# lms-07/LGTEUN

Hardware: AMD Instinct MI355X
Metric: train image-pairs/sec, GF-2 4-band 128x128, K=4, bs=32/GPU (higher is better)
Workload: dtype f32 (GEMMs and the local mixer: split 16-bit MFMA -- f16 pairs in the forward FFN, the W2 products of its backward and P V, bf16 triples elsewhere -- fp32 accumulate; fp32-equivalent); 1 GPU; BASELINE configs[1]: C=4, MS 32x32, PAN 128x128, K=4, 32 pairs/GPU, train step = fwd + L1 + bwd + Adam + StepLR tick; mode=faithful, global_batch=32, parallelism=dp1, dropout=True

## Files before the change

### include/lgteun_hip.h

```cpp
#ifndef LGTEUN_HIP_H
#define LGTEUN_HIP_H

#include <stddef.h>
#include <stdint.h>

#ifdef __cplusplus
extern "C" {
#endif

#define LG_TENSORS_SHARED 12
#define LG_TENSORS_PER_STAGE 119

#define LG_FLAG_FAITHFUL 1
#define LG_FLAG_SAVE 2
#define LG_FLAG_DROPOUT 4

#define LG_FLAG_BWD_LGT 8
#define LG_FLAG_BWD_DATA 16

#define LG_FLAG_CHAINED 32

#define LG_FLAG_DEFER_DEAD 64

#define LG_FLAG_STAGEWISE 128
// ... 83 lines not shown

int lg_optim_step_ex(float* params, const float* grads, float* state0, float* state1, float* state2, const int64_t* ranges,
                     int32_t n_ranges, int64_t max_range, int32_t step, int32_t algo, int32_t flags, double lr, double h0, double h1,
                     double eps, double weight_decay, double grad_scale, const float* clip_coef, float* ema, double ema_decay,
                     int32_t plain_adam, void* stream);

int lg_prof_enable(int32_t kernel_id, int32_t max_launches);
int lg_prof_reset(void);
void lg_prof_pause(int32_t paused);
int lg_prof_read(double* total_ms, int64_t* launches);
void lg_prof_disable(void);
const char* lg_kernel_name(int32_t kernel_id);

int lg_dropout_mask(uint64_t seed, int32_t stage, int32_t blk, int64_t first, int64_t n, float* out, void* stream);

int lg_op_resample(const float* x, float* y, int32_t planes, int32_t hi, int32_t wi, int32_t mode, void* stream);
int lg_op_data_step(const lg_plan* plan, const float* params, int32_t stage, const float* z_in, const float* ms,
                    const float* pan, float* z_out, float* tmp, int32_t B, void* stream);
int lg_op_lgt(const lg_plan* plan, const float* params, int32_t stage, const float* z, float* out, void* workspace,
              size_t workspace_bytes, int32_t B, int32_t flags, uint64_t seed, void* stream);
int lg_op_lgt_stages(const lg_plan* plan, const float* params, int32_t stage0, int32_t n, const float* z, float* out, void* workspace,
                     size_t workspace_bytes, int32_t B, int32_t flags, uint64_t seed, int32_t grid_cap, void* stream);
int lg_workspace_deadout(const lg_plan* plan, int32_t B, int32_t train, size_t* offset, size_t* stage_stride);
int lg_op_block(const lg_plan* plan, const float* params, int32_t stage, int32_t blk, int32_t which, const float* x,
                float* y, void* workspace, size_t workspace_bytes, int32_t B, void* stream);

int lg_op_block_bwd(const lg_plan* plan, const float* params, float* grads, int32_t stage, int32_t blk, int32_t which,
                    const float* x, const float* dy, float* dx, void* workspace, size_t workspace_bytes, int32_t B,
                    void* stream);

int lg_op_data_step_bwd(const lg_plan* plan, const float* params, float* grads, int32_t stage, const float* z_in, const float* ms,
                        const float* pan, const float* dz_out, float* dz_in, void* workspace, size_t workspace_bytes, int32_t B,
                        void* stream);
int lg_op_lgt_bwd(const lg_plan* plan, const float* params, float* grads, int32_t stage, const float* z, const float* dout, float* dz,
                  void* workspace, size_t workspace_bytes, int32_t B, int32_t flags, uint64_t seed, void* stream);

#define LG_IQA_PEAK 2047.5
#define LG_IQA_SSIM_TAPS 11
#define LG_IQA_SSIM_SIGMA 1.5
#define LG_IQA_Q_BLOCK 8
#define LG_IQA_RATIO 4
#define LG_IQA_QNR_BLOCK 32
#define LG_IQA_MTF_TAPS 41
#define LG_IQA_MTF_GAIN 0.15
#define LG_IQA_MAX_BANDS 16
size_t lg_iqa_workspace_bytes(int32_t B, int32_t C, int32_t H, int32_t W, int32_t no_ref);
// ... 31 lines not shown
```

### lgteun_amd/_lib.py

```python
import ctypes
import os
from ctypes import POINTER, c_char_p, c_double, c_float, c_int32, c_int64, c_size_t, c_uint64, c_void_p

_HERE = os.path.dirname(os.path.abspath(__file__))
LIB_PATH = os.environ.get('LGTEUN_HIP_LIB') or os.path.join(_HERE, '_lgteun_hip.so')

LG_FLAG_FAITHFUL = 1
LG_FLAG_SAVE = 2
LG_FLAG_DROPOUT = 4
LG_FLAG_BWD_LGT = 8
LG_FLAG_BWD_DATA = 16
LG_FLAG_CHAINED = 32
LG_FLAG_DEFER_DEAD = 64
LG_FLAG_STAGEWISE = 128
KERNEL_IDS = {n: i for i, n in enumerate(['none', 'ffn1', 'ffn', 'fft', 'attn', 'upfuse', 'down', 'embed', 'tail', 'datastep', 'ffn1_bwd',
                                           'ffn2_bwd', 'fft_bwd', 'attn_bwd', 'wgrad', 'batch', 'scene_gather', 'scene_blend'])}


class LgConfig(ctypes.Structure):
    _fields_ = [('C', c_int32), ('K', c_int32), ('H', c_int32), ('W', c_int32), ('precision', c_int32), ('variant', ctypes.c_uint32)]


LG_VAR_FFN_STRIP, LG_VAR_FFN_TILE, LG_VAR_FFN_XP = 1, 2, 3
LG_VAR_FFN_SAVE3, LG_VAR_FFN_SAVE5 = 1 << 2, 2 << 2
# ... 67 lines not shown
    'lgteun_forward': (c_int32, [c_void_p, c_void_p, c_void_p, c_void_p, c_void_p, c_void_p, c_size_t, c_int32, c_int32,
                                 c_uint64, c_void_p]),
    'lgteun_backward': (c_int32, [c_void_p, c_void_p, c_void_p, c_void_p, c_void_p, c_void_p, c_void_p, c_size_t, c_int32,
                                  c_int32, c_uint64, c_void_p]),
    'lgteun_dead_forward': (c_int32, [c_void_p, c_void_p, c_void_p, c_size_t, c_int32, c_int32, c_uint64, c_void_p]),
    'lg_l1_loss': (c_int32, [c_void_p, c_void_p, c_void_p, c_void_p, c_int64, c_int64, c_float, c_void_p]),
    'lg_adam_step': (c_int32, [c_void_p, c_void_p, c_void_p, c_void_p, c_void_p, c_int32, c_int64, c_int32, c_float, c_float,
                               c_float, c_float, c_float, c_void_p]),
    'lg_l2_loss': (c_int32, [c_void_p, c_void_p, c_void_p, c_void_p, c_int64, c_int64, c_float, c_void_p]),
    'lg_optim_step': (c_int32, [c_void_p, c_void_p, c_void_p, c_void_p, c_void_p, c_void_p, c_int32, c_int64, c_int32, c_int32, c_int32,
                                c_double, c_double, c_double, c_double, c_double, c_double, c_void_p]),
    'lg_grad_norm_workspace_bytes': (c_size_t, [c_int32, c_int64]),
    'lg_grad_norm': (c_int32, [c_void_p, c_void_p, c_int32, c_int64, c_double, c_void_p, c_void_p, c_size_t, c_void_p]),
    'lg_optim_step_ex': (c_int32, [c_void_p, c_void_p, c_void_p, c_void_p, c_void_p, c_void_p, c_int32, c_int64, c_int32, c_int32, c_int32,
                                   c_double, c_double, c_double, c_double, c_double, c_double, c_void_p, c_void_p, c_double, c_int32,
                                   c_void_p]),
    'lg_op_resample': (c_int32, [c_void_p, c_void_p, c_int32, c_int32, c_int32, c_int32, c_void_p]),
    'lg_op_data_step': (c_int32, [c_void_p, c_void_p, c_int32, c_void_p, c_void_p, c_void_p, c_void_p, c_void_p, c_int32,
                                  c_void_p]),
    'lg_op_lgt': (c_int32, [c_void_p, c_void_p, c_int32, c_void_p, c_void_p, c_void_p, c_size_t, c_int32, c_int32, c_uint64,
                            c_void_p]),
    'lg_op_lgt_stages': (c_int32, [c_void_p, c_void_p, c_int32, c_int32, c_void_p, c_void_p, c_void_p, c_size_t, c_int32, c_int32, c_uint64,
                                   c_int32, c_void_p]),
    'lg_workspace_deadout': (c_int32, [c_void_p, c_int32, c_int32, POINTER(c_size_t), POINTER(c_size_t)]),
    'lg_op_block': (c_int32, [c_void_p, c_void_p, c_int32, c_int32, c_int32, c_void_p, c_void_p, c_void_p, c_size_t, c_int32,
                              c_void_p]),
    'lg_dropout_mask': (c_int32, [c_uint64, c_int32, c_int32, c_int64, c_int64, c_void_p, c_void_p]),
    'lg_prof_enable': (c_int32, [c_int32, c_int32]),
    'lg_prof_reset': (c_int32, []),
    'lg_prof_pause': (None, [c_int32]),
    'lg_prof_read': (c_int32, [POINTER(ctypes.c_double), POINTER(c_int64)]),
    'lg_prof_disable': (None, []),
    'lg_kernel_name': (c_char_p, [c_int32]),
    'lg_op_data_step_bwd': (c_int32, [c_void_p, c_void_p, c_void_p, c_int32, c_void_p, c_void_p, c_void_p, c_void_p, c_void_p, c_void_p,
                                      c_size_t, c_int32, c_void_p]),
    'lg_op_lgt_bwd': (c_int32, [c_void_p, c_void_p, c_void_p, c_int32, c_void_p, c_void_p, c_void_p, c_void_p, c_size_t, c_int32, c_int32,
                                c_uint64, c_void_p]),
    'lg_op_block_bwd': (c_int32, [c_void_p, c_void_p, c_void_p, c_int32, c_int32, c_int32, c_void_p, c_void_p, c_void_p, c_void_p,
                                  c_size_t, c_int32, c_void_p]),
    'lg_iqa_workspace_bytes': (c_size_t, [c_int32, c_int32, c_int32, c_int32, c_int32]),
    'lg_iqa_ref': (c_int32, [c_void_p, c_void_p, c_void_p, c_int32, c_int32, c_int32, c_int32, c_float, c_void_p, c_size_t, c_void_p]),
    'lg_iqa_no_ref': (c_int32, [c_void_p, c_void_p, c_void_p, c_void_p, c_int32, c_int32, c_int32, c_int32, c_float, c_void_p, c_size_t,
                                c_void_p]),
    'lg_pyr_down2': (c_int32, [c_void_p, c_void_p, c_int64, c_int32, c_int32, c_int32, c_void_p]),
    'lg_batch_assemble': (c_int32, [c_void_p, c_void_p, c_void_p, c_void_p, c_int64, c_void_p, c_int64, c_void_p, c_void_p, c_void_p, c_void_p,
                                    c_void_p, c_int32, c_int32, c_int32, c_int32, c_int32, c_int32, c_int32, c_float, c_int32, c_float, c_void_p]),
# ... 34 lines not shown
```

### lgteun_amd/csrc/api.hip

```cpp
#include <stdarg.h>
#include <stdio.h>
#include <stdlib.h>
#include <string.h>
#include <math.h>
#include <atomic>
#include <mutex>

#pragma GCC visibility push(default)
#include "../../include/lgteun_hip.h"
#pragma GCC visibility pop

#include "kernels.h"
#include "workspace.h"
#include "backward.h"

static thread_local char g_err[512] = "";

void lg_set_error(const char* fmt, ...) {
    va_list ap;
    va_start(ap, fmt);
    vsnprintf(g_err, sizeof(g_err), fmt, ap);
    va_end(ap);
}

// ... 442 lines not shown
}

extern "C" int lg_op_lgt(const lg_plan* plan, const float* params, int32_t stage, const float* z, float* out, void* workspace,
                         size_t workspace_bytes, int32_t B, int32_t flags, uint64_t seed, void* stream) {
    if (!plan || !params || !z || !out || !workspace || stage < 0 || stage >= plan->cfg.K) { lg_set_error("op_lgt: invalid argument"); return -1; }
    const int train = (flags & LG_FLAG_SAVE) ? 1 : 0;
    if (workspace_bytes < lg_workspace_bytes(plan, B, train)) { lg_set_error("op_lgt: workspace too small"); return -3; }
    NetBufs nb;
    carve(plan, B, train, workspace, nb);
    return lgt_fwd(plan, params, stage, z, out, nb, B, flags, seed, (hipStream_t)stream);
}

extern "C" int lg_op_lgt_stages(const lg_plan* plan, const float* params, int32_t stage0, int32_t n, const float* z, float* out, void* workspace,
                                size_t workspace_bytes, int32_t B, int32_t flags, uint64_t seed, int32_t grid_cap, void* stream) {
    if (!plan || !params || !z || !out || !workspace || B <= 0 || stage0 < 0 || n < 1 || stage0 + n > plan->cfg.K || grid_cap < 0) { lg_set_error("op_lgt_stages: invalid argument"); return -1; }
    if (flags & ~LG_FLAG_DROPOUT) { lg_set_error("op_lgt_stages: only LG_FLAG_DROPOUT applies (nothing is saved)"); return -2; }
    if (n > 1 && (!plan->stage_batch || n > plan->cfg.K - 1)) { lg_set_error("op_lgt_stages: this plan runs one stage per pass (lg_plan_stage_batch), or n > K-1"); return -2; }
    if (workspace_bytes < lg_workspace_bytes(plan, B, 0)) { lg_set_error("op_lgt_stages: workspace too small"); return -3; }
    NetBufs nb;
    carve(plan, B, 0, workspace, nb);
    hipStream_t s = (hipStream_t)stream;
    if (int rc = prep_stages(plan, params, stage0, stage0 + n, nb, s)) return rc;
    return lgt_fwd(plan, params, stage0, z, out, nb, B, flags, seed, s, true, n, (long)B * plan->cfg.C * plan->cfg.H * plan->cfg.W, grid_cap);
}

extern "C" int lg_op_block(const lg_plan* plan, const float* params, int32_t stage, int32_t blk, int32_t which, const float* x,
                           float* y, void* workspace, size_t workspace_bytes, int32_t B, void* stream) {
    if (!plan || !params || !x || !y || !workspace || stage < 0 || stage >= plan->cfg.K || blk < 0 || blk > 4 || which < 0 || which > 2) {
        lg_set_error("op_block: invalid argument");
        return -1;
    }
    if (workspace_bytes < lg_workspace_bytes(plan, B, 0)) { lg_set_error("op_block: workspace too small"); return -3; }
    hipStream_t s = (hipStream_t)stream;
    NetBufs nb;
    carve(plan, B, 0, workspace, nb);
    BlockBufs bb = nb.blk[blk];
    int rc;
    const size_t npix = (size_t)B * bb.h * bb.w;
    if (which == 0 || which == 1) {
        if ((rc = launch_ln_split(bb.e, x, params + plan->blk(stage, blk, B_LN1G), params + plan->blk(stage, blk, B_LN1B), bb.g, B,
                                  bb.h * bb.w, s)))
            return rc;
    }
    if (which == 0) {
        FftArgs f;
        f.g = bb.g; f.o = y; f.amp = nullptr; f.pha = nullptr; f.sgn = nullptr; f.scratch = nb.fft_scratch;
// ... 467 lines not shown
```

### lgteun_amd/csrc/k_attn_m.hip

```cpp
#include "kernels.h"
#include "split_bf16.h"


namespace am {

__host__ __device__ constexpr int pw(int prod) { return prod == 0 ? 1 : prod == 1 ? 1 : prod == 2 ? 2 : prod == 3 ? 1 : prod == 4 ? 3 : 2; }
__host__ __device__ constexpr int px(int prod) { return prod == 0 ? 1 : prod == 1 ? 2 : prod == 2 ? 1 : prod == 3 ? 3 : prod == 4 ? 1 : 2; }
__host__ __device__ constexpr int pw2(int prod) { return prod == 0 ? 2 : 1; }
__host__ __device__ constexpr int px2(int prod) { return prod == 1 ? 2 : 1; }
__host__ __device__ constexpr int nprod(int np) { return np == 3 ? 6 : (np == 2 ? 3 : 1); }
template <int NP> __host__ __device__ constexpr int pwN(int prod) { return NP == 2 ? pw2(prod) : pw(prod); }
template <int NP> __host__ __device__ constexpr int pxN(int prod) { return NP == 2 ? px2(prod) : px(prod); }
__host__ __device__ constexpr int cdiv(int a, int b) { return (a + b - 1) / b; }

__device__ __forceinline__ float vmax2(float a, float b) { return fmaxf(a, b); }
__device__ __forceinline__ float vmax3(float a, float b, float c) { return fmaxf(fmaxf(a, b), c); }
__device__ __forceinline__ float xg_sum(float v) {
    u32x2_t r = __builtin_amdgcn_permlane32_swap(__float_as_uint(v), __float_as_uint(v), false, false);
    v = __uint_as_float(r.x) + __uint_as_float(r.y);
    r = __builtin_amdgcn_permlane16_swap(__float_as_uint(v), __float_as_uint(v), false, false);
    return __uint_as_float(r.x) + __uint_as_float(r.y);
}
__device__ __forceinline__ float xg_max(float v) {
    u32x2_t r = __builtin_amdgcn_permlane32_swap(__float_as_uint(v), __float_as_uint(v), false, false);
// ... 120 lines not shown

template <int HC>
struct Geo {
    static constexpr int E = 2 * HC, D = HC / 2, DG = D / 4;
    static constexpr int NCH = E / 16;
    static constexpr int NY = HC >= 16 ? HC / 16 : 1;
    static constexpr int MTQK = D / 4;
    static constexpr int NTV = HC >= 16 ? HC / 16 : 1;
    __host__ __device__ static constexpr int qk_oc(int mt, int r) {
        const int gq = r >> 2, idx = mt * 4 + (r & 3);
        const int isq = idx / (2 * DG), h = (idx / DG) % 2, dd = idx % DG;
        return (isq ? 0 : HC) + h * D + gq * DG + dd;
    }
    __host__ __device__ static constexpr int v_oc(int nt, int c) { return (HC == 8 && c >= 8) ? -1 : 2 * HC + 16 * nt + c; }
};

}

#ifdef LG_ATTN_STAMPS
__device__ unsigned long long am_stamps[1024][4][8];
#define AM_STAMP(i) do { __builtin_amdgcn_sched_barrier(0); const unsigned long long t__ = __builtin_amdgcn_s_memtime(); st[i] += t__ - tprev; tprev = t__; __builtin_amdgcn_sched_barrier(0); } while (0)
#else
#define AM_STAMP(i) do { } while (0)
#endif
template <int HC, int NP, bool MULTI = false>
__global__ __launch_bounds__(256, (HC <= 16 ? 2 : 1)) void k_attn_m(AttnArgs a_, int nwin, int nquads, int uneven) {
    using namespace am;
    using G = Geo<HC>;
    constexpr int E = G::E, D = G::D, DG = G::DG, NCH = G::NCH, NY = G::NY, MTQK = G::MTQK, NTV = G::NTV;
    constexpr int NPQ = NP == 2 ? 2 : NP, NPP = NP == 2 ? 3 : NP;
    constexpr int CHY = 4 * NY, NKQ = cdiv(nprod(NPQ) * CHY, 8);
    constexpr int NKS = cdiv(nprod(NPQ) * DG, 8);
    constexpr int CHC = 4 * NCH, NKP = cdiv(nprod(NPP) * CHC, 8);
    constexpr int MTP = NCH;
    constexpr int NPV = NP >= 2 ? 2 : 1;
    constexpr bool RELOADX = HC >= 32;
    constexpr float LOG2E = 1.44269504088896340736f;
    extern __shared__ __attribute__((aligned(16))) u32x4_t smem4[];
    float4* sPos = reinterpret_cast<float4*>(smem4);
    u32x4_t* sWqk = smem4 + 2 * 4 * 4 * 64;
    u32x4_t* sWv = sWqk + MTQK * NKQ * 64;
    u32x4_t* sWp = sWv + NTV * NKQ * 64;
    const int lane = threadIdx.x & 63, wave = threadIdx.x >> 6, g = lane >> 4, c = lane & 15;

#ifdef LG_ATTN_STAMPS
    unsigned long long st[8] = {0, 0, 0, 0, 0, 0, 0, 0}, tprev = __builtin_amdgcn_s_memtime();
#endif
    const StageSel sg = a_.sg;
    constexpr bool multi = MULTI;
    const int half = (int)gridDim.x >> 1, first = (int)blockIdx.x < half ? 1 : 0;
    const int nmine = uneven ? (first ? uneven : 8 - uneven) : 0x7fffffff;
    const int q0 = uneven ? (first ? (int)blockIdx.x : half * uneven + ((int)blockIdx.x - half)) : (int)blockIdx.x;
    const int qstep = multi ? 1 : (uneven ? half : (int)gridDim.x);
    const int per_stage = multi ? __builtin_amdgcn_readfirstlane(nquads / sg.n) : nquads;
    const int run0 = multi ? __builtin_amdgcn_readfirstlane((int)(blockIdx.x * (unsigned)nquads / gridDim.x)) : q0;
    const int run1 = multi ? __builtin_amdgcn_readfirstlane((int)((blockIdx.x + 1) * (unsigned)nquads / gridDim.x)) : nquads;
    int seg0 = run0;
    do {
    const int stg = multi ? __builtin_amdgcn_readfirstlane(seg0 / per_stage) : 0;
    const int seg1 = multi ? min(run1, (stg + 1) * per_stage) : run1;
    AttnArgs a = a_;
    {
        const long po = stg * sg.pstride;
        a.pos += po; a.ln1g += po; a.ln1b += po; a.qkvw += po; a.qkvb += po; a.projw += po; a.projb += po;
        if (NP == 2) a.scales += stg * sg.as_stride;
    }
    const uint64_t dseed = multi ? mix_seed(sg.seed, sg.stage0 + stg, sg.blk) : a.seed;
    const long dpix0 = (long)stg * sg.Bs * a.h * a.w;
    if (seg0 != run0) __syncthreads();
    float sy = 1.f, sw = 1.f, sq = 1.f, sk = 1.f;
    if (NP == 2) { sy = uniform_f(a.scales[0]); sw = uniform_f(a.scales[1]); sq = uniform_f(a.scales[2]); sk = uniform_f(a.scales[3]); }
    const float syw = sy * sw, inv_yw = 1.0f / syw, sqk = sq * sk, inv_qk = 1.0f / sqk;
    float4 pv[8];
#pragma unroll
    for (int j = 0; j < 8; ++j) {
        const int u = j * 256 + threadIdx.x, ln = u & 63, kt = (u >> 6) & 3, qt = (u >> 8) & 3, h = u >> 10;
        pv[j] = *reinterpret_cast<const float4*>(a.pos + ((h * 64 + 16 * qt + (ln & 15)) * 64 + 16 * kt + 4 * (ln >> 4)));
    }
    auto oc_qk = [](int t, int r) { return G::qk_oc(t, r); };
    auto oc_v = [](int t, int r) { return G::v_oc(t, r); };
    auto oc_p = [](int t, int r) { return 16 * t + r; };
    WStage<NPQ, CHY, NKQ, MTQK> wsq;
    WStage<NPQ, CHY, NKQ, NTV> wsv;
// ... 237 lines not shown
            for (int mt = 0; mt < MTP; ++mt) {
                f32x4_t acc = {bp[mt][0], bp[mt][1], bp[mt][2], bp[mt][3]};
#pragma unroll
                for (int k = 0; k < NKP; ++k) acc = mfma_bf(sWp[(mt * NKP + k) * 64 + lane], cf[k], acc);
                float o[4];
                const uint64_t di = (uint64_t)((pix - dpix0) * E + 16 * mt + 4 * g);
#pragma unroll
                for (int v = 0; v < 4; ++v) o[v] = acc[v];
                if (a.dropout) {
                    float s0, s1, s2, s3;
                    dropout_scale2(dseed, di, s0, s1);
                    dropout_scale2(dseed, di + 2, s2, s3);
                    o[0] *= s0; o[1] *= s1; o[2] *= s2; o[3] *= s3;
                }
                const float4 xr = RELOADX ? *reinterpret_cast<const float4*>(xw + (qt * tstep * E + 16 * mt + lx)) : xv[qt][mt];
                *reinterpret_cast<float4*>(yw + (qt * tstep * E + 16 * mt + lx)) = make_float4(xr.x + o[0], xr.y + o[1], xr.z + o[2], xr.w + o[3]);
            }
        }
        AM_STAMP(5);
    }
    seg0 = seg1;
    } while (MULTI && seg0 < run1);
#ifdef LG_ATTN_STAMPS
    if (lane == 0 && blockIdx.x < 1024) {
        for (int i = 0; i < 6; ++i) am_stamps[blockIdx.x][wave][i] = st[i];
        am_stamps[blockIdx.x][wave][7] = 1ull;
    }
#endif
}

template <int HC, int NP, bool MULTI = false>
static int launch_attn_m_t(const AttnArgs& a, hipStream_t s) {
    using G = am::Geo<HC>;
    constexpr int NPQ = NP == 2 ? 2 : NP, NPP = NP == 2 ? 3 : NP;
    constexpr int NKQ = am::cdiv(am::nprod(NPQ) * 4 * G::NY, 8), NKP = am::cdiv(am::nprod(NPP) * 4 * G::NCH, 8);
    const int nwin = a.B * (a.h / 8) * (a.w / 8);
    const int nquads = (nwin + 3) / 4;
    const size_t lds = (size_t)(2 * 4 * 4 * 64 + (G::MTQK + G::NTV) * NKQ * 64 + G::NCH * NKP * 64) * 16;
    static DeviceOnce attr_once;
    if (attr_once.need()) {
        hipError_t e = hipFuncSetAttribute((const void*)k_attn_m<HC, NP, MULTI>, hipFuncAttributeMaxDynamicSharedMemorySize, 160 * 1024);
        if (e != hipSuccess) { lg_set_error("attn_m: hipFuncSetAttribute: %s", hipGetErrorString(e)); return (int)e; }
        attr_once.done();
    }
    static std::atomic<int> per_cu_cache[64];
    int per_cu = per_cu_cache[DeviceOnce::dev()].load(std::memory_order_acquire);
    if (per_cu <= 0) {
        int nb = 0;
        hipError_t e = hipOccupancyMaxActiveBlocksPerMultiprocessor(&nb, (const void*)k_attn_m<HC, NP, MULTI>, 256, lds);
        if (e != hipSuccess || nb < 1) { lg_set_error("attn_m: occupancy query: %s (%d)", hipGetErrorString(e), nb); return e != hipSuccess ? (int)e : -3; }
        per_cu = nb;
        per_cu_cache[DeviceOnce::dev()].store(per_cu, std::memory_order_release);
    }
    int ncu = 256;
    const int cap = ncu * per_cu;
    const int rounds = (nquads + cap - 1) / cap;
    int grid = nquads < cap ? nquads : (nquads + rounds - 1) / rounds;
    constexpr bool multi = MULTI;
    if (multi) {
        if (a.save_o || a.save_l || a.sg.Bs <= 0 || a.B != a.sg.n * a.sg.Bs || (a.sg.Bs * (a.h / 8) * (a.w / 8)) % 4) { lg_set_error("attn_m: a window quad would straddle the stages of the launch"); return -2; }
        if (nquads > cap) grid = cap;
        if (a.sg.grid_cap > 0 && grid > a.sg.grid_cap) grid = a.sg.grid_cap;
    }
#ifndef LG_ATTN_UNEVEN
#define LG_ATTN_UNEVEN 5
#endif
    const int uneven = (!multi && per_cu == 2 && grid == 512 && nquads == 4 * grid && nwin == 4 * nquads) ? LG_ATTN_UNEVEN : 0;
    k_attn_m<HC, NP, MULTI><<<grid, 256, lds, s>>>(a, nwin, nquads, uneven == 4 ? 0 : uneven);
    LG_CHECK_LAUNCH();
    return 0;
}

int launch_attn_m(int e, const AttnArgs& a, hipStream_t s) {
    ProfScope prof__(LG_K_ATTN, s, a.sg.n);
    if ((a.h & 7) || (a.w & 7)) { lg_set_error("attn: h,w must be multiples of 8"); return -2; }
    if (a.sg.n > 1) {
        if (e == 16) return a.bf16 ? launch_attn_m_t<8, 1, true>(a, s) : (a.scales ? launch_attn_m_t<8, 2, true>(a, s) : launch_attn_m_t<8, 3, true>(a, s));
        if (e == 32) return a.bf16 ? launch_attn_m_t<16, 1, true>(a, s) : (a.scales ? launch_attn_m_t<16, 2, true>(a, s) : launch_attn_m_t<16, 3, true>(a, s));
        lg_set_error("attn: e=%d takes one stage per launch", e);
        return -2;
    }
    if (a.bf16) {
        if (e == 16) return launch_attn_m_t<8, 1>(a, s);
        if (e == 32) return launch_attn_m_t<16, 1>(a, s);
        if (e == 64) return launch_attn_m_t<32, 1>(a, s);
    } else if (a.scales) {
        if (e == 16) return launch_attn_m_t<8, 2>(a, s);
        if (e == 32) return launch_attn_m_t<16, 2>(a, s);
        if (e == 64) return launch_attn_m_t<32, 2>(a, s);
    } else {
        if (e == 16) return launch_attn_m_t<8, 3>(a, s);
// ... 7 lines not shown
```

### lgteun_amd/csrc/k_ffn_xr.hip

```cpp
#include "kernels.h"

#include "hstore.h"
#include "split_bf16.h"

#ifndef LG_XR_GRID
#define LG_XR_GRID 512
#endif
#ifdef LG_STAMPS
__device__ unsigned long long g_xr_stamps[512 * 4 * 10 * 8];
#define XSTAMP_AT(si_, i) do { unsigned long long t__; asm volatile("s_memtime %0\n\ts_waitcnt lgkmcnt(0)" : "=s"(t__)); \
                       g_xr_stamps[(((blockIdx.x & 511) * 4 + wave) * 10 + (si_)) * 8 + (i)] = t__; } while (0)
#define XSTAMP(i) do { unsigned long long t__; asm volatile("s_memtime %0\n\ts_waitcnt lgkmcnt(0)" : "=s"(t__)); \
                       g_xr_stamps[(((blockIdx.x & 511) * 4 + wave) * 10 + (stamp_si < 9 ? stamp_si : 9)) * 8 + (i)] = t__; } while (0)
extern "C" __attribute__((visibility("default"))) int lg_debug_xr_stamps(unsigned long long* host) {
    return (int)hipMemcpyFromSymbol(host, HIP_SYMBOL(g_xr_stamps), sizeof(g_xr_stamps));
}
#else
#define XSTAMP_AT(si_, i) do { } while (0)
#define XSTAMP(i) do { } while (0)
#endif

#ifndef LG_XR_TURN
#define LG_XR_TURN 0
#endif
#ifndef LG_XR_UNEVEN
#define LG_XR_UNEVEN 16
#endif
#define XR_TAKE_TURNS() do { if (LG_XR_TURN) { \
        const unsigned long long tt__ = __builtin_amdgcn_s_memtime(); \
        if ((((unsigned)(tt__ >> LG_XR_TURN)) ^ slot_par) & 1u) __builtin_amdgcn_s_setprio(3); else __builtin_amdgcn_s_setprio(0); } } while (0)
__device__ unsigned g_xr_turn[8192];

namespace xr {

constexpr int E = 16, N1 = 64, TX = 16, HX = 18, TY = 8, RING = 10, LDR = 68;
constexpr int NF1 = 8, NF2 = 16, NF3 = 4, NFRAG = NF1 + NF2 + NF3;
constexpr size_t OFF_W = 0;
constexpr size_t OFF_TAPS = OFF_W + (size_t)NFRAG * 64 * 16;
constexpr size_t OFF_PAR = OFF_TAPS + (size_t)N1 * 9 * 4;
constexpr int P_B1 = 0, P_B2 = 64, P_DWB = 128, P_B3 = 192, P_N1G = 208, P_N1B = 224, P_FLOATS = 240;
constexpr size_t OFF_RING = OFF_PAR + (size_t)P_FLOATS * 4;
constexpr size_t LDS_BYTES = OFF_RING + (size_t)RING * HX * LDR * 4;
static_assert(LDS_BYTES <= 80 * 1024, "two workgroups per CU");
static_assert(OFF_RING % 16 == 0 && OFF_TAPS % 16 == 0 && OFF_PAR % 16 == 0, "16-byte aligned LDS regions");

#ifndef LG_XR_NT
#define LG_XR_NT 0
#endif
#ifndef LG_XR_FENCES
// ... 63 lines not shown
template <int SAVE, int NP, bool MULTI = false>
__global__ __launch_bounds__(256) __attribute__((amdgpu_waves_per_eu(2))) void k_ffn_xr(Ffn1Args a1_, Ffn2Args a2_, int tiles_x, int strips_y, int nstrips,
                                                                                       int SH, int dS) {
    using namespace xr;
    extern __shared__ __attribute__((aligned(16))) unsigned char smem_raw[];
    float* ring = reinterpret_cast<float*>(smem_raw + OFF_RING);
    u32x4_t* sW = reinterpret_cast<u32x4_t*>(smem_raw + OFF_W);
    float* sTaps = reinterpret_cast<float*>(smem_raw + OFF_TAPS);
    float* sPar = reinterpret_cast<float*>(smem_raw + OFF_PAR);
    const int wave = threadIdx.x >> 6, lane = threadIdx.x & 63, g = lane >> 4, c_ = lane & 15, c = c_;
    const int uwave = __builtin_amdgcn_readfirstlane(wave);
    unsigned slot_par = 0;
    if (LG_XR_TURN) {
        const unsigned hw = __builtin_amdgcn_s_getreg((12 - 1) << 11 | 4 << 6 | 4);
        const unsigned xcc = __builtin_amdgcn_s_getreg((3 - 1) << 11 | 0 << 6 | 20);
        const unsigned key = (xcc << 10) | (((hw >> 9) & 7u) << 7) | (((hw >> 8) & 1u) << 6) | (((hw >> 4) & 15u) << 2) | (hw & 3u);
        unsigned old_ = 0;
        if (lane == 0) old_ = atomicXor(&g_xr_turn[key & 8191u], 1u);
        slot_par = (unsigned)__builtin_amdgcn_readfirstlane((int)old_) & 1u;
    }
    const int h = a2_.h, w = a2_.w;
    const StageSel sg = a1_.sg;
    constexpr bool multi = MULTI;
    const int per_stage = multi ? sg.Bs * tiles_x * strips_y : nstrips;
    const int run0 = multi ? __builtin_amdgcn_readfirstlane((int)(blockIdx.x * (unsigned)nstrips / gridDim.x)) : (int)blockIdx.x;
    const int run1 = multi ? __builtin_amdgcn_readfirstlane((int)((blockIdx.x + 1) * (unsigned)nstrips / gridDim.x)) : nstrips;
    const int rstep = multi ? 1 : (int)gridDim.x;
    int seg0 = run0;
    do {
    const int st = multi ? __builtin_amdgcn_readfirstlane(seg0 / per_stage) : 0;
    const int seg1 = multi ? min(run1, (st + 1) * per_stage) : run1;
    Ffn1Args a1 = a1_;
    Ffn2Args a2 = a2_;
    {
        const long po = st * sg.pstride;
        a1.ln2g += po; a1.ln2b += po; a1.w1 += po; a1.b1 += po; a1.w2 += po; a1.b2 += po;
        a2.dww += po; a2.dwb += po; a2.w3 += po; a2.b3 += po;
        if (a2.g) { a2.n1g += po; a2.n1b += po; }
        if (NP == 2) a1.scales += st * sg.fs_stride;
    }
    if (seg0 != run0) __syncthreads();
    constexpr bool BF = NP == 1;
    float sx = 1.f, sa1 = 1.f, sa3 = 1.f, sw1 = 1.f, sw2 = 1.f, sw3 = 1.f;
    if (NP == 2) { sx = uniform_f(a1.scales[0]); sa1 = uniform_f(a1.scales[1]); sa3 = uniform_f(a1.scales[2]); sw1 = uniform_f(a1.scales[3]); sw2 = uniform_f(a1.scales[4]); sw3 = uniform_f(a1.scales[5]); }
    const float S1 = sx * sw1, S2 = sa1 * sw2, S3 = sa3 * sw3;
    const float inv2 = 1.0f / S2, inv3 = 1.0f / S3;
#ifdef LG_XR_OLDGELU
    const xr::GKold gk1 = {0.70710678118654752440f / S1, 0.5f * sa1 / S1}, gk3 = {0.70710678118654752440f, 0.5f * sa3};
#else
    const GeluK gk1 = gelu_k(0.70710678118654752440f / S1, 0.5f * sa1 / S1), gk3 = gelu_k(0.70710678118654752440f, 0.5f * sa3);
#endif

    auto strip_geo = [&](int strip, int& tx_i, long& b, int& Y0, int& Yend) {
        if (dS) {
// ... 485 lines not shown
                        if (ok && g >= 2) {
#endif
                            const long hw = (long)h * w, sp = (long)y * w + x;
                            float* dst = a2.g + (b * (E / 2) + (4 * g - E / 2)) * hw + sp;
                            dst[0] = d0 * rstd * ng.x + nbv.x;
                            dst[hw] = d1 * rstd * ng.y + nbv.y;
                            dst[2 * hw] = d2 * rstd * ng.z + nbv.z;
                            dst[3 * hw] = d3 * rstd * ng.w + nbv.w;
                        }
                    }
                    XR_FENCE();
                }
            }
            XSTAMP(4);
            __syncthreads();
            XR_TAKE_TURNS();
            XSTAMP(5);
        }
    }
    seg0 = seg1;
    } while (MULTI && seg0 < run1);
}

int launch_ffn_xr(const Ffn1Args& a1, const Ffn2Args& a2, hipStream_t s) {
    using namespace xr;
    ProfScope prof__(LG_K_FFN2, s, a1.sg.n);
    static DeviceOnce attr_once;
    if (attr_once.need()) {
        hipError_t e = hipFuncSetAttribute((const void*)k_ffn_xr<0, 2>, hipFuncAttributeMaxDynamicSharedMemorySize, (int)LDS_BYTES);
        if (e == hipSuccess) e = hipFuncSetAttribute((const void*)k_ffn_xr<3, 2>, hipFuncAttributeMaxDynamicSharedMemorySize, (int)LDS_BYTES);
        if (e == hipSuccess) e = hipFuncSetAttribute((const void*)k_ffn_xr<0, 1>, hipFuncAttributeMaxDynamicSharedMemorySize, (int)LDS_BYTES);
        if (e == hipSuccess) e = hipFuncSetAttribute((const void*)k_ffn_xr<3, 1>, hipFuncAttributeMaxDynamicSharedMemorySize, (int)LDS_BYTES);
        if (e == hipSuccess) e = hipFuncSetAttribute((const void*)k_ffn_xr<0, 2, true>, hipFuncAttributeMaxDynamicSharedMemorySize, (int)LDS_BYTES);
        if (e == hipSuccess) e = hipFuncSetAttribute((const void*)k_ffn_xr<0, 1, true>, hipFuncAttributeMaxDynamicSharedMemorySize, (int)LDS_BYTES);
        if (e != hipSuccess) { lg_set_error("ffn_xr: hipFuncSetAttribute: %s", hipGetErrorString(e)); return (int)e; }
        attr_once.done();
    }
    if (!a1.hbf && !a1.scales) { lg_set_error("ffn_xr: the f16-pair instance needs the operand scales"); return -2; }
    const bool save = a1.h2 != nullptr;
    if (save && (a1.a1s || a1.g1s || a2.g3s)) { lg_set_error("ffn_xr: saves h2 / h3 (or h2 alone: a3s null, the backward re-computes h3) only"); return -2; }
    if ((long)a2.B * a2.h * a2.w * N1 >= (1ll << 32)) { lg_set_error("ffn_xr: hidden tensor of %ld elements exceeds the 32-bit save index", (long)a2.B * a2.h * a2.w * N1); return -2; }
    const int tiles_x = (a2.w + 15) / 16;
    const bool multi = a1.sg.n > 1;
    const int Bsh = multi ? a1.sg.Bs : a2.B;
    if (multi && (save || a1.sg.Bs <= 0 || a2.B != a1.sg.n * a1.sg.Bs)) { lg_set_error("ffn_xr: B = %d is not %d stages of %d samples", a2.B, a1.sg.n, a1.sg.Bs); return -2; }
    int SH = (a2.h + 7) / 8 * 8;
    while (SH > 16 && (long)Bsh * tiles_x * ((a2.h + SH - 1) / SH) < LG_XR_GRID) SH = (SH / 2 + 7) / 8 * 8;
    const int strips_y = (a2.h + SH - 1) / SH;
    const int nstrips = a2.B * tiles_x * strips_y;
    int grid = nstrips < LG_XR_GRID ? nstrips : LG_XR_GRID;
    if (multi && a1.sg.grid_cap > 0 && grid > a1.sg.grid_cap) grid = a1.sg.grid_cap;
    int dS = 0;
    if (!multi && LG_XR_UNEVEN && nstrips == LG_XR_GRID && LG_XR_GRID == 512 && (strips_y & 1) == 0 && SH >= 32 && a2.h % (2 * SH) == 0) dS = (SH * LG_XR_UNEVEN / 64 + 7) / 8 * 8;
    if (a1.hbf) {
        if (save) k_ffn_xr<3, 1><<<grid, 256, LDS_BYTES, s>>>(a1, a2, tiles_x, strips_y, nstrips, SH, dS);
        else if (multi) k_ffn_xr<0, 1, true><<<grid, 256, LDS_BYTES, s>>>(a1, a2, tiles_x, strips_y, nstrips, SH, dS);
        else k_ffn_xr<0, 1><<<grid, 256, LDS_BYTES, s>>>(a1, a2, tiles_x, strips_y, nstrips, SH, dS);
    } else if (save) k_ffn_xr<3, 2><<<grid, 256, LDS_BYTES, s>>>(a1, a2, tiles_x, strips_y, nstrips, SH, dS);
    else if (multi) k_ffn_xr<0, 2, true><<<grid, 256, LDS_BYTES, s>>>(a1, a2, tiles_x, strips_y, nstrips, SH, dS);
    else k_ffn_xr<0, 2><<<grid, 256, LDS_BYTES, s>>>(a1, a2, tiles_x, strips_y, nstrips, SH, dS);
    LG_CHECK_LAUNCH();
    return 0;
}
```

### lgteun_amd/csrc/kernels.h

```cpp
#pragma once
#include "common.h"

int launch_pyr_down2(const void* pan, float* pan_l, int64_t planes, int H, int W, int dtype, hipStream_t s);
int launch_batch_assemble(const void* pan, const void* lr, const void* mul, const float* pan_l, int64_t N, const int32_t* idx, int64_t idx_offset,
                          const uint32_t* flips, float* o_pan, float* o_lr, float* o_mul, float* o_pan_l, int B, int C, int H, int W, int h, int w,
                          int dtype, float divisor, int n_div, float post_scale, hipStream_t s);
int launch_window_assemble(const void* pan, const void* lr, const void* mul, const int32_t* origins, int64_t n_windows, int64_t first,
                           const uint32_t* flips, float* o_pan, float* o_lr, float* o_mul, float* o_pan_l, int B, int C, int Hs, int Ws, int P, int Q,
                           int dtype, float divisor, int n_div, float post_scale, hipStream_t s);
int launch_fir_decimate4(const void* in, void* out, const double* taps, int64_t planes, int H, int W, int n_taps, int phase, int dtype, int out_f32,
                         hipStream_t s);
int launch_scene_gather(const void* pan, const void* ms, const int32_t* origins, int64_t n_tiles, int64_t first, float* o_pan, float* o_ms,
                        int B, int C, int H, int W, int th, int tw, int dtype, float divisor, int n_div, float post_scale, hipStream_t s);
int launch_scene_blend(const float* tiles, float* scene, int64_t first, int B, int C, int H, int W, int th, int tw, int overlap, hipStream_t s);
int launch_scene_to_u16(const float* src, uint16_t* dst, int64_t n, float scale, hipStream_t s);
size_t iqa_workspace_bytes(int B, int C, int H, int W, int no_ref);
int launch_iqa_ref(const float* pred, const float* gt, double* out, int B, int C, int H, int W, float scale, void* workspace,
                   size_t workspace_bytes, hipStream_t s);
int launch_iqa_no_ref(const float* pred, const float* pan, const float* ms, double* out, int B, int C, int H, int W, float scale,
                      void* workspace, size_t workspace_bytes, hipStream_t s);
size_t grad_norm_workspace_bytes(int n_ranges, int64_t max_range);
int launch_grad_norm(const float* grads, const int64_t* ranges, int n_ranges, int64_t max_range, double max_norm, float* out, void* workspace,
                     size_t workspace_bytes, hipStream_t s);

// ... 22 lines not shown
    float *t1, *r, *s1;
    float* pr;
    const float *d1w, *d1b, *d3w, *d3b, *dt1w, *dt1b, *dt3w, *dt3b, *rw, *rb, *rtw, *rtb, *eta;
    int B, C, N;
};
bool dstep_fused_ok(int C, int H, int W);
int launch_dstep_fwd(const DstepFwdArgs& a, hipStream_t s);

struct StageSel {
    int n = 1;
    int Bs = 0;
    long pstride = 0;
    long zstride = 0;
    int fs_stride = 0;
    int as_stride = 0;
    long ws_stride = 0;
    int grid_cap = 0;
    uint64_t seed = 0;
    int stage0 = 0, blk = 0;
};
#ifdef __HIPCC__
__device__ __forceinline__ int stage_of(const StageSel& sg, int b) { return sg.n > 1 ? __builtin_amdgcn_readfirstlane(b / sg.Bs) : 0; }
__device__ __forceinline__ int stage_of_unit(const StageSel& sg, int unit, int per_sample) { return sg.n > 1 ? __builtin_amdgcn_readfirstlane(unit / (per_sample * sg.Bs)) : 0; }
#endif

struct EmbedArgs {
    const float* z;
    float* x;
    float* g;
    const float *dww, *dwb, *w, *b, *lng, *lnb, *n1g, *n1b;
    int HW;
    long total;
    StageSel sg;
};
int launch_embed(int C, const EmbedArgs& a, hipStream_t s);

struct DownArgs {
    const float* x;
    float* y;
    float* g;
    float* u_save;
    const float *w, *b, *n1g, *n1b;
    int B, H, W;
    StageSel sg;
};
int launch_down(int E, const DownArgs& a, hipStream_t s);

// ... 107 lines not shown
```

Measured before the change: 6463 image-pairs/sec.

## Extend uneven two-half work splits to multi-stage attention and FFN launches

Moves the grid-geometry logic of the windowed attention and the strip FFN into shared helper functions. It then enables, for chained multi-stage launches, the uneven split already used by single-stage launches: workgroups in the first and second halves of the grid take different-sized chunks (or strip-height pairs). The aim is to balance co-resident workgroups on each CU and trim tail time. It also re-derives lane indices inside the stage loop behind an opaque asm barrier for large head counts, to steer register allocation, and adds debug entry points that report the split. The new indexing, including stage offsets for the second half, adds correctness risk.

After: 6566 image-pairs/sec, median of 6. +1.6%, better.

```diff
diff --git a/include/lgteun_hip.h b/include/lgteun_hip.h
--- a/include/lgteun_hip.h
+++ b/include/lgteun_hip.h
@@ -129,6 +129,8 @@
 int lg_op_lgt_stages(const lg_plan* plan, const float* params, int32_t stage0, int32_t n, const float* z, float* out, void* workspace,
                      size_t workspace_bytes, int32_t B, int32_t flags, uint64_t seed, int32_t grid_cap, void* stream);
 int lg_workspace_deadout(const lg_plan* plan, int32_t B, int32_t train, size_t* offset, size_t* stage_stride);
+int lg_debug_stage_runs(int32_t kind, int32_t units, int32_t per_stage, int32_t grid, int32_t split, int32_t* out, int32_t n_out);
+int lg_debug_stage_decision(int32_t kind, int32_t h, int32_t w, int32_t Bs, int32_t n, int32_t grid_cap, int32_t* out8);
 int lg_op_block(const lg_plan* plan, const float* params, int32_t stage, int32_t blk, int32_t which, const float* x,
                 float* y, void* workspace, size_t workspace_bytes, int32_t B, void* stream);
 
diff --git a/lgteun_amd/_lib.py b/lgteun_amd/_lib.py
--- a/lgteun_amd/_lib.py
+++ b/lgteun_amd/_lib.py
@@ -113,6 +113,8 @@
                             c_void_p]),
     'lg_op_lgt_stages': (c_int32, [c_void_p, c_void_p, c_int32, c_int32, c_void_p, c_void_p, c_void_p, c_size_t, c_int32, c_int32, c_uint64,
                                    c_int32, c_void_p]),
+    'lg_debug_stage_runs': (c_int32, [c_int32, c_int32, c_int32, c_int32, c_int32, POINTER(c_int32), c_int32]),
+    'lg_debug_stage_decision': (c_int32, [c_int32, c_int32, c_int32, c_int32, c_int32, c_int32, POINTER(c_int32)]),
     'lg_workspace_deadout': (c_int32, [c_void_p, c_int32, c_int32, POINTER(c_size_t), POINTER(c_size_t)]),
     'lg_op_block': (c_int32, [c_void_p, c_void_p, c_int32, c_int32, c_int32, c_void_p, c_void_p, c_void_p, c_size_t, c_int32,
                               c_void_p]),
diff --git a/lgteun_amd/csrc/api.hip b/lgteun_amd/csrc/api.hip
--- a/lgteun_amd/csrc/api.hip
+++ b/lgteun_amd/csrc/api.hip
@@ -488,6 +488,44 @@
     hipStream_t s = (hipStream_t)stream;
     if (int rc = prep_stages(plan, params, stage0, stage0 + n, nb, s)) return rc;
     return lgt_fwd(plan, params, stage0, z, out, nb, B, flags, seed, s, true, n, (long)B * plan->cfg.C * plan->cfg.H * plan->cfg.W, grid_cap);
+}
+
+extern "C" int lg_debug_stage_runs(int32_t kind, int32_t units, int32_t per_stage, int32_t grid, int32_t split, int32_t* out, int32_t n_out) {
+    if (kind < 0 || kind > 1 || units <= 0 || per_stage <= 0 || units % per_stage || grid <= 0 || !out || n_out < 0 || (int64_t)units * grid >= (1ll << 31)) {
+        lg_set_error("debug_stage_runs: invalid argument");
+        return -1;
+    }
+    const bool uneven = kind == 0 ? split != 0 : split != 4;
+    if (!uneven && grid > units) { lg_set_error("debug_stage_runs: more workgroups than units"); return -1; }
+    if (uneven && ((grid & 1) || (kind == 0 ? 2 * units < grid : units < grid) || (kind == 1 && (split < 1 || split > 7)))) { lg_set_error("debug_stage_runs: an uneven split needs an even grid, a unit per workgroup and 1 <= eighths <= 7"); return -2; }
+    int rows = 0;
+    for (int wg = 0; wg < grid; ++wg) {
+        const StageRun r = !uneven ? stage_run_even(units, grid, wg) : (kind == 0 ? stage_run_pairs(units, grid, wg) : stage_run_chunk(units, grid, wg, split));
+        int seg0 = r.run0;
+        do {
+            const int st = seg0 / per_stage, seg1 = stage_seg_end(st, r.run1, per_stage);
+            if (rows < n_out) { int32_t* o = out + 5 * (size_t)rows; o[0] = wg; o[1] = seg0; o[2] = seg1; o[3] = st; o[4] = r.base; }
+            ++rows;
+            seg0 = seg1;
+        } while (seg0 < r.run1);
+    }
+    return rows;
+}
+
+extern "C" int lg_debug_stage_decision(int32_t kind, int32_t h, int32_t w, int32_t Bs, int32_t n, int32_t grid_cap, int32_t* out8) {
+    if ((kind != 0 && kind != 8 && kind != 16) || h <= 0 || w <= 0 || Bs <= 0 || n < 1 || grid_cap < 0 || !out8 || (int64_t)Bs * n * h * w >= (1ll << 31)) { lg_set_error("debug_stage_decision: invalid argument"); return -1; }
+    if (kind == 0) {
+        const XrGeo q = ffn_xr_geometry(h, w, Bs * n, Bs, n, grid_cap);
+        const int sh = q.dS ? 1 : 0;
+        const int32_t o[8] = {q.dS != 0, q.dS, q.nstrips >> sh, (Bs * q.tiles_x * q.strips_y) >> sh, q.grid, q.SH, q.tiles_x, q.strips_y};
+        memcpy(out8, o, sizeof(o));
+    } else {
+        if ((h & 7) || (w & 7) || (Bs * (h / 8) * (w / 8)) % 4) { lg_set_error("debug_stage_decision: not whole window quads per stage"); return -2; }
+        const AttnMGeo q = attn_m_geometry(kind, h, w, Bs * n, n, grid_cap, 2);
+        const int32_t o[8] = {q.uneven != 0, q.uneven ? q.uneven : 4, q.nquads, q.nquads / n, q.grid, q.nwin, 0, 0};
+        memcpy(out8, o, sizeof(o));
+    }
+    return 0;
 }
 
 extern "C" int lg_op_block(const lg_plan* plan, const float* params, int32_t stage, int32_t blk, int32_t which, const float* x,
diff --git a/lgteun_amd/csrc/k_attn_m.hip b/lgteun_amd/csrc/k_attn_m.hip
--- a/lgteun_amd/csrc/k_attn_m.hip
+++ b/lgteun_amd/csrc/k_attn_m.hip
@@ -166,6 +166,9 @@
 #define AM_STAMP(i) do { __builtin_amdgcn_sched_barrier(0); const unsigned long long t__ = __builtin_amdgcn_s_memtime(); st[i] += t__ - tprev; tprev = t__; __builtin_amdgcn_sched_barrier(0); } while (0)
 #else
 #define AM_STAMP(i) do { } while (0)
+#endif
+#ifndef LG_ATTN_MULTI_REFORM_HC
+#define LG_ATTN_MULTI_REFORM_HC 16
 #endif
 template <int HC, int NP, bool MULTI = false>
 __global__ __launch_bounds__(256, (HC <= 16 ? 2 : 1)) void k_attn_m(AttnArgs a_, int nwin, int nquads, int uneven) {
@@ -185,7 +188,6 @@
     u32x4_t* sWqk = smem4 + 2 * 4 * 4 * 64;
     u32x4_t* sWv = sWqk + MTQK * NKQ * 64;
     u32x4_t* sWp = sWv + NTV * NKQ * 64;
-    const int lane = threadIdx.x & 63, wave = threadIdx.x >> 6, g = lane >> 4, c = lane & 15;
 
 #ifdef LG_ATTN_STAMPS
     unsigned long long st[8] = {0, 0, 0, 0, 0, 0, 0, 0}, tprev = __builtin_amdgcn_s_memtime();
@@ -193,16 +195,20 @@
     const StageSel sg = a_.sg;
     constexpr bool multi = MULTI;
     const int half = (int)gridDim.x >> 1, first = (int)blockIdx.x < half ? 1 : 0;
-    const int nmine = uneven ? (first ? uneven : 8 - uneven) : 0x7fffffff;
+    const int nmine = (!multi && uneven) ? (first ? uneven : 8 - uneven) : 0x7fffffff;
     const int q0 = uneven ? (first ? (int)blockIdx.x : half * uneven + ((int)blockIdx.x - half)) : (int)blockIdx.x;
     const int qstep = multi ? 1 : (uneven ? half : (int)gridDim.x);
     const int per_stage = multi ? __builtin_amdgcn_readfirstlane(nquads / sg.n) : nquads;
-    const int run0 = multi ? __builtin_amdgcn_readfirstlane((int)(blockIdx.x * (unsigned)nquads / gridDim.x)) : q0;
-    const int run1 = multi ? __builtin_amdgcn_readfirstlane((int)((blockIdx.x + 1) * (unsigned)nquads / gridDim.x)) : nquads;
+    const StageRun rn = stage_run_chunk(nquads, (int)gridDim.x, (int)blockIdx.x, multi ? uneven : 0);
+    const int run0 = multi ? __builtin_amdgcn_readfirstlane(rn.run0) : q0;
+    const int run1 = multi ? __builtin_amdgcn_readfirstlane(rn.run1) : nquads;
     int seg0 = run0;
     do {
     const int stg = multi ? __builtin_amdgcn_readfirstlane(seg0 / per_stage) : 0;
-    const int seg1 = multi ? min(run1, (stg + 1) * per_stage) : run1;
+    const int seg1 = multi ? stage_seg_end(stg, run1, per_stage) : run1;
+    int tid_ = threadIdx.x;
+    if (MULTI && HC >= LG_ATTN_MULTI_REFORM_HC) asm volatile("" : "+v"(tid_));
+    const int lane = tid_ & 63, wave = tid_ >> 6, g = lane >> 4, c = lane & 15;
     AttnArgs a = a_;
     {
         const long po = stg * sg.pstride;
@@ -486,11 +492,41 @@
     seg0 = seg1;
     } while (MULTI && seg0 < run1);
 #ifdef LG_ATTN_STAMPS
+    const int lane = threadIdx.x & 63, wave = threadIdx.x >> 6;
     if (lane == 0 && blockIdx.x < 1024) {
         for (int i = 0; i < 6; ++i) am_stamps[blockIdx.x][wave][i] = st[i];
         am_stamps[blockIdx.x][wave][7] = 1ull;
     }
 #endif
+}
+
+#ifndef LG_ATTN_UNEVEN
+#define LG_ATTN_UNEVEN 5
+#endif
+#ifndef LG_ATTN_MULTI_UNEVEN
+#define LG_ATTN_MULTI_UNEVEN 5
+#endif
+#ifndef LG_ATTN_MULTI_UNEVEN16
+#define LG_ATTN_MULTI_UNEVEN16 4
+#endif
+AttnMGeo attn_m_geometry(int HC, int h, int w, int B, int n, int grid_cap, int per_cu) {
+    AttnMGeo q;
+    q.nwin = B * (h / 8) * (w / 8);
+    q.nquads = (q.nwin + 3) / 4;
+    const int ncu = 256;
+    const int cap = ncu * per_cu;
+    const int rounds = (q.nquads + cap - 1) / cap;
+    q.grid = q.nquads < cap ? q.nquads : (q.nquads + rounds - 1) / rounds;
+    const bool multi = n > 1;
+    bool capped = false;
+    if (multi) {
+        if (q.nquads > cap) q.grid = cap;
+        if (grid_cap > 0 && q.grid > grid_cap) { q.grid = grid_cap; capped = true; }
+    }
+    int u = (!multi && per_cu == 2 && q.grid == 512 && q.nquads == 4 * q.grid && q.nwin == 4 * q.nquads) ? LG_ATTN_UNEVEN : 0;
+    if (multi && per_cu == 2 && q.grid == 2 * ncu && !capped && q.nquads >= 2 * ncu && (HC == 8 || HC == 16)) u = HC == 8 ? LG_ATTN_MULTI_UNEVEN : LG_ATTN_MULTI_UNEVEN16;
+    q.uneven = u == 4 ? 0 : u;
+    return q;
 }
 
 template <int HC, int NP, bool MULTI = false>
@@ -498,8 +534,6 @@
     using G = am::Geo<HC>;
     constexpr int NPQ = NP == 2 ? 2 : NP, NPP = NP == 2 ? 3 : NP;
     constexpr int NKQ = am::cdiv(am::nprod(NPQ) * 4 * G::NY, 8), NKP = am::cdiv(am::nprod(NPP) * 4 * G::NCH, 8);
-    const int nwin = a.B * (a.h / 8) * (a.w / 8);
-    const int nquads = (nwin + 3) / 4;
     const size_t lds = (size_t)(2 * 4 * 4 * 64 + (G::MTQK + G::NTV) * NKQ * 64 + G::NCH * NKP * 64) * 16;
     static DeviceOnce attr_once;
     if (attr_once.need()) {
@@ -516,21 +550,11 @@
         per_cu = nb;
         per_cu_cache[DeviceOnce::dev()].store(per_cu, std::memory_order_release);
     }
-    int ncu = 256;
-    const int cap = ncu * per_cu;
-    const int rounds = (nquads + cap - 1) / cap;
-    int grid = nquads < cap ? nquads : (nquads + rounds - 1) / rounds;
     constexpr bool multi = MULTI;
-    if (multi) {
-        if (a.save_o || a.save_l || a.sg.Bs <= 0 || a.B != a.sg.n * a.sg.Bs || (a.sg.Bs * (a.h / 8) * (a.w / 8)) % 4) { lg_set_error("attn_m: a window quad would straddle the stages of the launch"); return -2; }
-        if (nquads > cap) grid = cap;
-        if (a.sg.grid_cap > 0 && grid > a.sg.grid_cap) grid = a.sg.grid_cap;
-    }
-#ifndef LG_ATTN_UNEVEN
-#define LG_ATTN_UNEVEN 5
-#endif
-    const int uneven = (!multi && per_cu == 2 && grid == 512 && nquads == 4 * grid && nwin == 4 * nquads) ? LG_ATTN_UNEVEN : 0;
-    k_attn_m<HC, NP, MULTI><<<grid, 256, lds, s>>>(a, nwin, nquads, uneven == 4 ? 0 : uneven);
+    if (multi && (a.save_o || a.save_l || a.sg.Bs <= 0 || a.B != a.sg.n * a.sg.Bs || (a.sg.Bs * (a.h / 8) * (a.w / 8)) % 4)) { lg_set_error("attn_m: a window quad would straddle the stages of the launch"); return -2; }
+    const AttnMGeo geo = attn_m_geometry(HC, a.h, a.w, a.B, multi ? a.sg.n : 1, a.sg.grid_cap, per_cu);
+    const int nwin = geo.nwin, nquads = geo.nquads, grid = geo.grid, uneven = geo.uneven;
+    k_attn_m<HC, NP, MULTI><<<grid, 256, lds, s>>>(a, nwin, nquads, uneven);
     LG_CHECK_LAUNCH();
     return 0;
 }
diff --git a/lgteun_amd/csrc/k_ffn_xr.hip b/lgteun_amd/csrc/k_ffn_xr.hip
--- a/lgteun_amd/csrc/k_ffn_xr.hip
+++ b/lgteun_amd/csrc/k_ffn_xr.hip
@@ -25,6 +25,9 @@
 #endif
 #ifndef LG_XR_UNEVEN
 #define LG_XR_UNEVEN 16
+#endif
+#ifndef LG_XR_MULTI_UNEVEN
+#define LG_XR_MULTI_UNEVEN 16
 #endif
 #define XR_TAKE_TURNS() do { if (LG_XR_TURN) { \
         const unsigned long long tt__ = __builtin_amdgcn_s_memtime(); \
@@ -134,14 +137,17 @@
     const int h = a2_.h, w = a2_.w;
     const StageSel sg = a1_.sg;
     constexpr bool multi = MULTI;
-    const int per_stage = multi ? sg.Bs * tiles_x * strips_y : nstrips;
-    const int run0 = multi ? __builtin_amdgcn_readfirstlane((int)(blockIdx.x * (unsigned)nstrips / gridDim.x)) : (int)blockIdx.x;
-    const int run1 = multi ? __builtin_amdgcn_readfirstlane((int)((blockIdx.x + 1) * (unsigned)nstrips / gridDim.x)) : nstrips;
+    const bool pairs = multi && dS != 0;
+    const int per_stage = multi ? (sg.Bs * tiles_x * strips_y) >> (pairs ? 1 : 0) : nstrips;
+    const StageRun rn = stage_run_halves(nstrips >> (pairs ? 1 : 0), (int)gridDim.x >> (pairs ? 1 : 0), (int)blockIdx.x);
+    const int run0 = multi ? __builtin_amdgcn_readfirstlane(rn.run0 + rn.base) : (int)blockIdx.x;
+    const int run1 = multi ? __builtin_amdgcn_readfirstlane(rn.run1 + rn.base) : nstrips;
     const int rstep = multi ? 1 : (int)gridDim.x;
     int seg0 = run0;
     do {
-    const int st = multi ? __builtin_amdgcn_readfirstlane(seg0 / per_stage) : 0;
-    const int seg1 = multi ? min(run1, (st + 1) * per_stage) : run1;
+    const int sq = multi ? __builtin_amdgcn_readfirstlane(seg0 / per_stage) : 0;
+    const int st = sq >= sg.n ? sq - sg.n : sq;
+    const int seg1 = multi ? stage_seg_end(sq, run1, per_stage) : run1;
     Ffn1Args a1 = a1_;
     Ffn2Args a2 = a2_;
     {
@@ -673,6 +679,26 @@
     } while (MULTI && seg0 < run1);
 }
 
+XrGeo ffn_xr_geometry(int h, int w, int B, int Bs, int n, int grid_cap) {
+    XrGeo q;
+    q.tiles_x = (w + 15) / 16;
+    const bool multi = n > 1;
+    const int Bsh = multi ? Bs : B;
+    int SH = (h + 7) / 8 * 8;
+    while (SH > 16 && (long)Bsh * q.tiles_x * ((h + SH - 1) / SH) < LG_XR_GRID) SH = (SH / 2 + 7) / 8 * 8;
+    q.SH = SH;
+    q.strips_y = (h + SH - 1) / SH;
+    q.nstrips = B * q.tiles_x * q.strips_y;
+    q.grid = q.nstrips < LG_XR_GRID ? q.nstrips : LG_XR_GRID;
+    const bool capped = multi && grid_cap > 0 && q.grid > grid_cap;
+    if (capped) q.grid = grid_cap;
+    q.dS = 0;
+    const bool shape_ok = LG_XR_GRID == 512 && (q.strips_y & 1) == 0 && SH >= 32 && h % (2 * SH) == 0;
+    if (!multi && LG_XR_UNEVEN && q.nstrips == LG_XR_GRID && shape_ok) q.dS = (SH * LG_XR_UNEVEN / 64 + 7) / 8 * 8;
+    if (multi && LG_XR_MULTI_UNEVEN && !capped && q.grid == LG_XR_GRID && (q.grid & 1) == 0 && shape_ok) q.dS = (SH * LG_XR_MULTI_UNEVEN / 64 + 7) / 8 * 8;
+    return q;
+}
+
 int launch_ffn_xr(const Ffn1Args& a1, const Ffn2Args& a2, hipStream_t s) {
     using namespace xr;
     ProfScope prof__(LG_K_FFN2, s, a1.sg.n);
@@ -691,18 +717,10 @@
     const bool save = a1.h2 != nullptr;
     if (save && (a1.a1s || a1.g1s || a2.g3s)) { lg_set_error("ffn_xr: saves h2 / h3 (or h2 alone: a3s null, the backward re-computes h3) only"); return -2; }
     if ((long)a2.B * a2.h * a2.w * N1 >= (1ll << 32)) { lg_set_error("ffn_xr: hidden tensor of %ld elements exceeds the 32-bit save index", (long)a2.B * a2.h * a2.w * N1); return -2; }
-    const int tiles_x = (a2.w + 15) / 16;
     const bool multi = a1.sg.n > 1;
-    const int Bsh = multi ? a1.sg.Bs : a2.B;
     if (multi && (save || a1.sg.Bs <= 0 || a2.B != a1.sg.n * a1.sg.Bs)) { lg_set_error("ffn_xr: B = %d is not %d stages of %d samples", a2.B, a1.sg.n, a1.sg.Bs); return -2; }
-    int SH = (a2.h + 7) / 8 * 8;
-    while (SH > 16 && (long)Bsh * tiles_x * ((a2.h + SH - 1) / SH) < LG_XR_GRID) SH = (SH / 2 + 7) / 8 * 8;
-    const int strips_y = (a2.h + SH - 1) / SH;
-    const int nstrips = a2.B * tiles_x * strips_y;
-    int grid = nstrips < LG_XR_GRID ? nstrips : LG_XR_GRID;
-    if (multi && a1.sg.grid_cap > 0 && grid > a1.sg.grid_cap) grid = a1.sg.grid_cap;
-    int dS = 0;
-    if (!multi && LG_XR_UNEVEN && nstrips == LG_XR_GRID && LG_XR_GRID == 512 && (strips_y & 1) == 0 && SH >= 32 && a2.h % (2 * SH) == 0) dS = (SH * LG_XR_UNEVEN / 64 + 7) / 8 * 8;
+    const XrGeo geo = ffn_xr_geometry(a2.h, a2.w, a2.B, a1.sg.Bs, a1.sg.n, a1.sg.grid_cap);
+    const int tiles_x = geo.tiles_x, strips_y = geo.strips_y, nstrips = geo.nstrips, SH = geo.SH, grid = geo.grid, dS = geo.dS;
     if (a1.hbf) {
         if (save) k_ffn_xr<3, 1><<<grid, 256, LDS_BYTES, s>>>(a1, a2, tiles_x, strips_y, nstrips, SH, dS);
         else if (multi) k_ffn_xr<0, 1, true><<<grid, 256, LDS_BYTES, s>>>(a1, a2, tiles_x, strips_y, nstrips, SH, dS);
diff --git a/lgteun_amd/csrc/kernels.h b/lgteun_amd/csrc/kernels.h
--- a/lgteun_amd/csrc/kernels.h
+++ b/lgteun_amd/csrc/kernels.h
@@ -68,7 +68,30 @@
 #ifdef __HIPCC__
 __device__ __forceinline__ int stage_of(const StageSel& sg, int b) { return sg.n > 1 ? __builtin_amdgcn_readfirstlane(b / sg.Bs) : 0; }
 __device__ __forceinline__ int stage_of_unit(const StageSel& sg, int unit, int per_sample) { return sg.n > 1 ? __builtin_amdgcn_readfirstlane(unit / (per_sample * sg.Bs)) : 0; }
+
+struct StageRun { int run0, run1, base; };
+__host__ __device__ inline StageRun stage_run_halves(int units, int half, int wg) {
+    const int first = wg < half ? 1 : 0, j = wg - (first ? 0 : half);
+    return {(int)((unsigned)j * (unsigned)units / (unsigned)half), (int)(((unsigned)j + 1u) * (unsigned)units / (unsigned)half), first ? 0 : units};
+}
+__host__ __device__ inline StageRun stage_run_even(int units, int grid, int wg) { return stage_run_halves(units, grid, wg); }
+__host__ __device__ inline StageRun stage_run_pairs(int npairs, int grid, int wg) { return stage_run_halves(npairs, grid >> 1, wg); }
+__host__ __device__ inline StageRun stage_run_chunk(int units, int grid, int wg, int u) {
+    const StageRun ch = stage_run_halves(units, u ? grid >> 1 : grid, wg);
+    if (!u) return ch;
+    const int len = ch.run1 - ch.run0;
+    int n1 = (len * u + 4) >> 3;
+    n1 = n1 > len - 1 ? len - 1 : n1;
+    n1 = n1 < 1 ? 1 : n1;
+    return ch.base ? StageRun{ch.run0 + n1, ch.run1, 0} : StageRun{ch.run0, ch.run0 + n1, 0};
+}
+__host__ __device__ inline int stage_seg_end(int st, int run1, int per_stage) { return run1 < (st + 1) * per_stage ? run1 : (st + 1) * per_stage; }
 #endif
+
+struct XrGeo { int tiles_x, SH, strips_y, nstrips, grid, dS; };
+XrGeo ffn_xr_geometry(int h, int w, int B, int Bs, int n, int grid_cap);
+struct AttnMGeo { int nwin, nquads, grid, uneven; };
+AttnMGeo attn_m_geometry(int HC, int h, int w, int B, int n, int grid_cap, int per_cu);
 
 struct EmbedArgs {
     const float* z;
```
